# bergmanlab/TELR

Measured on AMD Instinct MI355X. Metric: gbp_aligned_per_s, higher is better.
Workload: dtype int16

## Files before the change

telr_amd/csrc/kernels.hip.h:

```cpp
#pragma once
#include <hip/hip_runtime.h>
#include <stdint.h>

#define TELR_NEG      (-(1 << 28))
#include "part_plan.h"
#define SK_TILE       1024
#define SK_THREADS    256
#define DP_DMAX       4096

struct ChainOpt {
    int32_t max_gap, bw, min_cnt, min_chain_score, chain_gap_q8, chain_skip_q8;
    int32_t dense_n, dense_span, mw_n;
};
struct DpOpt {
    int32_t a, b, q, e, q2, e2, sc_ambi, zdrop;
    int32_t cx_scale, cx_open, cx_emax, cx_emin, cx_dec, cx_flat;
};
__host__ __device__ __forceinline__ int d_cx_ext(const DpOpt &o, int len) { int v = o.cx_emax - o.cx_dec * len; return v > o.cx_emin ? v : o.cx_emin; }
__host__ __device__ __forceinline__ int d_cx_cost(const DpOpt &o, int L)
{
    int t = o.cx_open;
    for (int i = 0; i < L && i < o.cx_flat; ++i) t += d_cx_ext(o, i);
    if (L > o.cx_flat) t += (L - o.cx_flat) * o.cx_emin;
    return t;
// ... 1563 lines not shown
            const uint32_t qi = (klo >> 8) & 0xffffffu, sp = klo & 0xffu;
            const int32_t gpos = (int32_t)(gi & 0x7fffffffu);
            const int lo = i - CHAIN_SCAN_H > 0 ? i - CHAIN_SCAN_H : 0;
            int32_t best = (int32_t)sp, bp = -1, nskip = 0;
            for (int c = 0; ; ++c) {
                const int jt = i - 1 - 64 * c, j = jt - lane;
                if (jt < lo) break;
                uint32_t g = wg, q = wq; int32_t fj2p2 = wf, pj = wp; bool mk = false;
                if (c > 0 && j >= lo) {
                    const uint64_t k = a[j];
                    g = (uint32_t)(k >> 32); q = (uint32_t)A_Q(k);
                    fj2p2 = 2 * f[base + j] + 2;
                    const int32_t pa = p[base + j];
                    pj = pa >= 0 ? pa - pdelta : -1;
                    mk = mark[base + j] == (int32_t)(base + i);
                }
                const bool inw = j >= lo && ((g ^ gi) >> 31) == 0u && gpos - (int32_t)(g & 0x7fffffffu) <= (int32_t)max_gap;
                bool ok;
                const int32_t v2 = d_chain_link<SKIP>(gi, qi, sp - 1u, g + 1u, q + 1u, fj2p2, max_gap, ddc, gap_q8, skip_q8, ok);
                const bool valid = inw && ok;
                const int32_t v = v2 >> 1;
                const uint32_t u = valid && v > best ? (uint32_t)(v - best) : 0u;
                const uint32_t pre = d_wave_scan_max0(u);
                const uint32_t ex = (uint32_t)__shfl_up((int)pre, 1);
                const bool imp = u > (lane ? ex : 0u);
                fl[lane] = 0;
                const int tl = jt - pj;
                if (valid && pj >= 0 && tl < 64) fl[tl] = 1;
                __builtin_amdgcn_fence(__ATOMIC_SEQ_CST, "wavefront");
                mk = mk || fl[lane] != 0;
                __builtin_amdgcn_fence(__ATOMIC_SEQ_CST, "wavefront");
                const int32_t s = valid ? (imp ? -1 : (mk ? 1 : 0)) : 0;
                const int32_t T = nskip + (int32_t)d_wave_scan_add((uint32_t)s);
                const int32_t x = T + (int32_t)d_wave_scan_max0(T < 0 ? (uint32_t)(-T) : 0u);
                const uint64_t brk = __ballot(x > CHAIN_SCAN_SKIP);
                const int b = brk ? __ffsll((unsigned long long)brk) - 1 : 64;
                const uint64_t scanned = b == 64 ? ~0ULL : ((1ULL << b) - 1);
                const uint64_t im = __ballot(imp) & scanned;
                if (im) {
                    const int hl = 63 - __clzll((long long)im);
                    best += (int32_t)__builtin_amdgcn_readlane((int)u, hl);
                    bp = jt - hl;
                }
                const uint64_t win = __ballot(inw);
                const bool more = b == 64 && win == ~0ULL && jt - 64 >= lo;
                if (!more) break;
                if (valid && pj >= 0 && tl >= 64) mark[base + pj] = (int32_t)(base + i);
                nskip = __builtin_amdgcn_readlane(x, 63);
                __threadfence_block();
            }
            of = lane == ii ? best : of; op = lane == ii ? bp : op;
            wg = (uint32_t)__shfl_up((int)wg, 1); wq = (uint32_t)__shfl_up((int)wq, 1); wf = __shfl_up(wf, 1); wp = __shfl_up(wp, 1);
            if (lane == 0) { wg = gi; wq = qi; wf = 2 * best + 2; wp = bp; }
        }
        if (lane < m) {
            f[base + i0 + lane] = of; p[base + i0 + lane] = op >= 0 ? op + pdelta : -1;
            mark[base + i0 + lane] = -1;
        }
        __threadfence_block();
        kb = kn;
    }
}
template <bool SKIP>
__global__ void __launch_bounds__(64) k_chain_scan(const uint64_t *__restrict__ keys, const int32_t *__restrict__ q_aoff, int32_t nq,
                                                   ChainOpt o, int32_t *__restrict__ f, int32_t *__restrict__ p, int32_t *__restrict__ mark,
                                                   const int32_t *__restrict__ q_order)
{
    __shared__ uint8_t fl[64];
    if ((int)blockIdx.x >= nq) return;
    const int q = q_order ? q_order[blockIdx.x] : blockIdx.x;
    d_chain_run_scan<SKIP>(keys, q_aoff[q], q_aoff[q + 1] - q_aoff[q], 0, o, f, p, mark, fl);
}
template <bool SKIP>
__global__ void __launch_bounds__(64) k_chain_scan_isl(const uint64_t *__restrict__ keys, const int32_t *__restrict__ isl_off, const int32_t *__restrict__ isl_pd,
                                                       const int32_t *__restrict__ nisl, ChainOpt o, int32_t *__restrict__ f, int32_t *__restrict__ p,
                                                       int32_t *__restrict__ mark)
{
    __shared__ uint8_t fl[64];
    const int n_isl = *nisl;
    for (int s = blockIdx.x; s < n_isl; s += gridDim.x)
        d_chain_run_scan<SKIP>(keys, isl_off[s], isl_off[s + 1] - isl_off[s], isl_pd[s], o, f, p, mark, fl);
}

__global__ void k_nonpeak(const int32_t *__restrict__ q_aoff, const int32_t *__restrict__ f, const int32_t *__restrict__ p, uint8_t *__restrict__ nonpeak)
{
    const int q = blockIdx.x;
    const int64_t base = q_aoff[q]; const int n = q_aoff[q + 1] - q_aoff[q];
    for (int i = threadIdx.x; i < n; i += blockDim.x) {
        int pj = p[base + i];
        if (pj >= 0 && f[base + i] > f[base + pj]) nonpeak[base + pj] = 1;
    }
}
__global__ void k_peaks(const int32_t *__restrict__ q_aoff, const int32_t *__restrict__ f, const uint8_t *__restrict__ nonpeak,
                        int32_t min_sc, uint64_t *__restrict__ pk, int32_t *__restrict__ n_peaks, int32_t *__restrict__ pk_end)
{
    __shared__ int32_t cnt;
    const int q = blockIdx.x;
    const int64_t base = q_aoff[q]; const int n = q_aoff[q + 1] - q_aoff[q];
    if (threadIdx.x == 0) cnt = 0;
    __syncthreads();
    for (int i = threadIdx.x; i < n; i += blockDim.x) {
        if (!nonpeak[base + i] && f[base + i] >= min_sc) {
            int s = atomicAdd(&cnt, 1);
            pk[base + s] = (uint64_t)(uint32_t)(0x7fffffff - f[base + i]) << 32 | (uint32_t)i;
        }
    }
    __syncthreads();
    if (threadIdx.x == 0) { n_peaks[q] = cnt; pk_end[q] = (int32_t)base + cnt; }
}

struct ChainRec { int32_t score, cnt, a_off, pad; uint64_t a0, a1; };


#define BT_INF 0xffffffffu
#define BT_RING 512
#define BT_RING_SCAN 8192
__global__ void k_bt_rank(const int32_t *__restrict__ q_aoff, const uint64_t *__restrict__ pk, const int32_t *__restrict__ n_peaks, uint32_t *__restrict__ owner)
{
    const int q = blockIdx.x;
    const int64_t base = q_aoff[q]; const int np = n_peaks[q];
    for (int t = threadIdx.x; t < np; t += blockDim.x) owner[base + (uint32_t)(pk[base + t] & 0xffffffffu)] = (uint32_t)t;
}
template <int RING>
__global__ void __launch_bounds__(64) k_bt_owner(const int32_t *__restrict__ q_aoff, int32_t nq, const int32_t *__restrict__ p, int32_t lookback,
                                                 uint32_t *__restrict__ owner, const int32_t *__restrict__ q_order)
{
    __shared__ uint32_t W[RING];
    __shared__ int32_t UP[64];
    const int q = q_order ? q_order[blockIdx.x] : blockIdx.x, lane = threadIdx.x;
    const int64_t base = q_aoff[q]; const int n = q_aoff[q + 1] - q_aoff[q];
    if (n <= 0) return;
    const int nblk = (n + 63) >> 6;
    for (int blk = nblk - 1; blk >= 0; --blk) {
        const int b0 = blk << 6;
        if (blk == nblk - 1) { for (int x = b0 - lookback + lane; x < b0 + 64; x += 64) if (x >= 0 && x < n) W[x & (RING - 1)] = owner[base + x]; }
        else { const int x = b0 - lookback + lane; if (x >= 0) W[x & (RING - 1)] = owner[base + x]; }
        const int i = b0 + lane; const bool valid = i < n;
        const int pi = valid ? p[base + i] : -1;
        int up = pi >= b0 ? pi - b0 : -1;
        UP[lane] = up;
        for (int k = 0; k < 6; ++k) {
            if (__ballot(up >= 0) == 0) break;
            if (up >= 0) atomicMin(&W[(b0 + up) & (RING - 1)], W[i & (RING - 1)]);
            const int nup = up >= 0 ? UP[up] : -1;
            UP[lane] = nup; up = nup;
        }
        if (valid) {
            const uint32_t v = W[i & (RING - 1)];
            owner[base + i] = v;
            if (pi >= 0 && pi < b0) atomicMin(&W[pi & (RING - 1)], v);
        }
    }
}
template <int RING>
__global__ void __launch_bounds__(64) k_bt_depth(const int32_t *__restrict__ q_aoff, int32_t nq, const int32_t *__restrict__ p, const uint32_t *__restrict__ owner,
                                                 int32_t *__restrict__ depth, int32_t *__restrict__ ch_top, const int32_t *__restrict__ q_order)
{
    __shared__ uint32_t OWN[RING];
    __shared__ int32_t DEP[RING];
    __shared__ int32_t UP[64], VAL[64];
    const int q = q_order ? q_order[blockIdx.x] : blockIdx.x, lane = threadIdx.x;
    const int64_t base = q_aoff[q]; const int n = q_aoff[q + 1] - q_aoff[q];
    const int nblk = (n + 63) >> 6;
    for (int blk = 0; blk < nblk; ++blk) {
        const int b0 = blk << 6, i = b0 + lane; const bool valid = i < n;
        const uint32_t o = valid ? owner[base + i] : BT_INF;
        const int pi = valid ? p[base + i] : -1;
        OWN[i & (RING - 1)] = o;
        const uint32_t po = pi >= 0 ? OWN[pi & (RING - 1)] : BT_INF;
        const bool conn = o != BT_INF && pi >= 0 && po == o;
        int up = -1, val = 0;
        if (conn) { if (pi >= b0) { up = pi - b0; val = 1; } else val = DEP[pi & (RING - 1)] + 1; }
        UP[lane] = up; VAL[lane] = val;
        for (int k = 0; k < 6; ++k) {
            if (__ballot(up >= 0) == 0) break;
            const int add = up >= 0 ? VAL[up] : 0, nup = up >= 0 ? UP[up] : -1;
            val += add;
            VAL[lane] = val; UP[lane] = nup; up = nup;
        }
        DEP[i & (RING - 1)] = val;
        if (valid) {
            depth[base + i] = val;
            if (o != BT_INF && !conn) ch_top[base + o] = i;
        }
    }
}
__global__ void __launch_bounds__(64) k_bt_emit(const uint64_t *__restrict__ keys, const int32_t *__restrict__ q_aoff, int32_t nq, const int32_t *__restrict__ f,
                                                const int32_t *__restrict__ p, const uint64_t *__restrict__ pk, const int32_t *__restrict__ n_peaks,
                                                const int32_t *__restrict__ ch_off, int32_t min_sc, int32_t min_cnt, const uint32_t *__restrict__ owner,
                                                const int32_t *__restrict__ depth, const int32_t *__restrict__ ch_top, int32_t *__restrict__ ch_aoff,
                                                ChainRec *__restrict__ rec, int32_t *__restrict__ n_chains, const int32_t *__restrict__ q_order)
{
    const int q = q_order ? q_order[blockIdx.x] : blockIdx.x, lane = threadIdx.x;
    const int64_t base = q_aoff[q]; const int np = n_peaks[q];
    ChainRec *out = rec + ch_off[q];
    int nch = 0, wr = 0;
    for (int t0 = 0; t0 < np; t0 += 64) {
        const int t = t0 + lane;
        bool keep = false; int cnt = 0, sc = 0, idx = 0, top = 0;
        if (t < np) {
            const uint64_t key = pk[base + t];
            idx = (int)(uint32_t)(key & 0xffffffffu);
            const int fi = 0x7fffffff - (int)(uint32_t)(key >> 32);
            if (owner[base + idx] == (uint32_t)t) {
                cnt = depth[base + idx] + 1;
                top = ch_top[base + t];
                const int pj = p[base + top];
                sc = fi - (pj >= 0 ? f[base + pj] : 0);
                keep = sc >= min_sc && cnt >= min_cnt;
            }
        }
        const uint64_t km = __ballot(keep);
        const int before = __popcll(km & ((1ULL << lane) - 1));
        int ps = keep ? cnt : 0;
#pragma unroll
        for (int d = 1; d < 64; d <<= 1) { const int v = __shfl_up(ps, d); if (lane >= d) ps += v; }
        if (t < np) ch_aoff[base + t] = keep ? wr + ps - cnt : -1;
        if (keep) {
            ChainRec r; r.score = sc; r.cnt = cnt; r.a_off = wr + ps - cnt; r.pad = 0;
            r.a0 = keys[base + top]; r.a1 = keys[base + idx];
            out[nch + before] = r;
        }
        nch += __popcll(km); wr += __shfl(ps, 63);
    }
    if (lane == 0) n_chains[q] = nch;
}
__global__ void k_bt_scatter(const uint64_t *__restrict__ keys, const int32_t *__restrict__ q_aoff, const uint32_t *__restrict__ owner, const int32_t *__restrict__ depth,
                             const int32_t *__restrict__ ch_aoff, uint64_t *__restrict__ canch, const int32_t *__restrict__ q_order)
{
    const int q = q_order ? q_order[blockIdx.x] : blockIdx.x;
    const int64_t base = q_aoff[q]; const int n = q_aoff[q + 1] - q_aoff[q];
    for (int i = threadIdx.x; i < n; i += blockDim.x) {
        const uint32_t o = owner[base + i];
        if (o == BT_INF) continue;
        const int ao = ch_aoff[base + o];
        if (ao >= 0) canch[base + ao + depth[base + i]] = keys[base + i];
    }
}

struct KeptChain {
    int32_t qid, tid, rev, cnt;
    int64_t a_glob;
    int32_t rs, qs, re, qe;
    int32_t qlen, tlen;
    int64_t qbase, tbase;
    uint32_t goff; int32_t pad;
};

struct SelOpt { float mask_level, pri_ratio; int32_t best_n, secondary, per_target; };
struct KeptLite { int32_t qid, score, cnt, rev, tid, rs, re, qs, qe, pad; };
__global__ void k_sel_keys(const int32_t *__restrict__ ch_off, const int32_t *__restrict__ n_chains, const ChainRec *__restrict__ rec,
                           uint64_t *__restrict__ key, int32_t *__restrict__ seg_end)
{
    const int q = blockIdx.x;
    const int base = ch_off[q], n = n_chains[q];
    for (int c = threadIdx.x; c < n; c += blockDim.x) key[base + c] = (uint64_t)(uint32_t)(0x7fffffff - rec[base + c].score) << 32 | (uint32_t)c;
    if (threadIdx.x == 0) seg_end[q] = base + n;
}
__device__ __forceinline__ void d_chain_box(const ChainRec &r, const uint32_t *__restrict__ goff, int n_targets, int &rev, int &tid, int &rs, int &re, int &qs, int &qe)
{
    rev = (int)(r.a0 >> 63);
    tid = d_tid_of(goff, n_targets, (uint32_t)A_G(r.a0));
    const int go = (int)goff[tid];
    rs = A_G(r.a0) - go - A_SPAN(r.a0) + 1; re = A_G(r.a1) - go + 1;
    if (rs < 0) rs = 0;
    qs = A_Q(r.a0) - A_SPAN(r.a0) + 1;      qe = A_Q(r.a1) + 1;
}
#define SEL_PCAP 1024
__global__ void __launch_bounds__(64) k_select1(const int32_t *__restrict__ ch_off, const int32_t *__restrict__ n_chains, const ChainRec *__restrict__ rec,
                                                const uint64_t *__restrict__ skey, const int32_t *__restrict__ qlen_of, const uint32_t *__restrict__ goff, int32_t n_targets,
                                                SelOpt o, int32_t *__restrict__ pfs, int32_t *__restrict__ pfe, int32_t *__restrict__ ptid, int32_t *__restrict__ pkey,
                                                int32_t *__restrict__ tcnt_t, int32_t *__restrict__ tcnt_n, uint8_t *__restrict__ keep, int32_t *__restrict__ n_kept,
                                                const int32_t *__restrict__ q_order)
{
    __shared__ int32_t Lfs[SEL_PCAP], Lfe[SEL_PCAP], Ltid[SEL_PCAP], Lkey[SEL_PCAP];
    const int q = q_order ? q_order[blockIdx.x] : blockIdx.x, lane = threadIdx.x;
    const int base = ch_off[q], n = n_chains[q], qlen = qlen_of[q];
    int n_prim = 0, n2_all = 0, n_t = 0, nk = 0;
    for (int i0 = 0; i0 < n; i0 += 64) {
        const int cnt = n - i0 < 64 ? n - i0 : 64;
        int my_fs = 0, my_fe = 0, my_tid = 0, my_sc = 0;
        if (lane < cnt) {
            const ChainRec r = rec[base + (int)(uint32_t)(skey[base + i0 + lane] & 0xffffffffu)];
            int rev, rs, re, qs, qe;
            d_chain_box(r, goff, n_targets, rev, my_tid, rs, re, qs, qe);
            my_fs = rev ? qlen - qe : qs; my_fe = rev ? qlen - qs : qe; my_sc = r.score;
        }
        bool my_keep = false;
        for (int u = 0; u < cnt; ++u) {
            const int fs = __builtin_amdgcn_readlane(my_fs, u), fe = __builtin_amdgcn_readlane(my_fe, u), tid = __builtin_amdgcn_readlane(my_tid, u),
                      sc = __builtin_amdgcn_readlane(my_sc, u);
            int parent = -1;
            for (int c0 = 0; c0 < n_prim && parent < 0; c0 += 64) {
                const int j = c0 + lane;
                bool hit = false;
                if (j < n_prim) {
                    const int jt = j < SEL_PCAP ? Ltid[j] : ptid[base + j];
                    if (!o.per_target || jt == tid) {
                        const int js = j < SEL_PCAP ? Lfs[j] : pfs[base + j], je = j < SEL_PCAP ? Lfe[j] : pfe[base + j];
                        const int lo = fs > js ? fs : js, hi = fe < je ? fe : je;
                        const int ol = hi > lo ? hi - lo : 0;
                        const int mn = (fe - fs) < (je - js) ? (fe - fs) : (je - js);
                        hit = (float)ol > o.mask_level * (float)mn;
                    }
                }
                const uint64_t m = __ballot(hit);
                if (m) parent = c0 + __ffsll((unsigned long long)m) - 1;
            }
            bool kp;
            if (parent < 0) {
                if (lane == 0) {
                    if (n_prim < SEL_PCAP) { Lfs[n_prim] = fs; Lfe[n_prim] = fe; Ltid[n_prim] = tid; Lkey[n_prim] = sc; }
                    else { pfs[base + n_prim] = fs; pfe[base + n_prim] = fe; ptid[base + n_prim] = tid; pkey[base + n_prim] = sc; }
                }
// ... 1916 lines not shown
```

telr_amd/csrc/telr_engine.hip:

```cpp
#include <hip/hip_runtime.h>
#include <cstring>
#include <string.h>
#include <rocprim/rocprim.hpp>
#include <algorithm>
#include <atomic>
#include <immintrin.h>
#include <chrono>
#include <cmath>
#include <condition_variable>
#include <cstdio>
#include <cstdlib>
#include <cstring>
#include <map>
#include <memory>
#include <mutex>
#include <string>
#include <thread>
#include <sys/mman.h>
#include <vector>
#include "../../include/telr_hip.h"
#include "kernels.hip.h"
#include "range_plan.h"
#include "sam_records.h"
#define TELR_HAVE_SEED_ARGS 1
// ... 1486 lines not shown
                          int32_t n_over, const int32_t *d_overlist, const int32_t *d_qorder, int32_t *d_f, int32_t *d_p)
{
    ChainOpt co; co.max_gap = mo->max_gap; co.bw = mo->bw_long > mo->bw ? mo->bw_long : mo->bw; co.min_cnt = mo->min_cnt; co.min_chain_score = mo->min_chain_score;
    co.chain_gap_q8 = mo->chain_gap_q8; co.chain_skip_q8 = mo->chain_skip_q8;
    static const bool chain_push = ab_on("chain_push"), chain_lazy = ab_on("chain_lazy"), chain_no_mw = ab_on("chain_no_mw");
    static int dense_v[3] = {2048, 48, 1 << 19};
    static const bool dense_env = [] { if (const char *e = getenv("TELR_CHAIN_DENSE")) sscanf(e, "%d%*[,:]%d%*[,:]%d", &dense_v[0], &dense_v[1], &dense_v[2]); return true; }();
    (void)dense_env;
    const int Rr = mo->chain_lookback / 64;
    const bool mw_all = dense_v[2] <= SEGSORT_CAP;
    static const bool no_islands = ab_on("no_islands");
    const bool islands = nq <= CHAIN_ISL_NQ && na > 0 && !no_islands;
    const bool mw = !(mo->flags & TELR_MF_CHAIN_SKIP) && !chain_push && !chain_lazy && !chain_no_mw && Rr >= 2 && na > 0 && !islands && dense_v[2] > 0 && (mw_all || n_over > 0);
    co.dense_n = dense_v[0]; co.dense_span = dense_v[1]; co.mw_n = mw ? dense_v[2] : 0;
#define CHAIN_LAUNCH(RR, SK) do { if (chain_push) hipLaunchKernelGGL((k_chain<RR, SK, 0>), dim3(nq), dim3(64), 0, st, d_skeys, d_qaoff, nq, co, d_f, d_p, d_qorder, 0); \
                                  else if (chain_lazy) hipLaunchKernelGGL((k_chain<RR, SK, 1>), dim3(nq), dim3(64), 0, st, d_skeys, d_qaoff, nq, co, d_f, d_p, d_qorder, 0); \
                                  else hipLaunchKernelGGL((k_chain<RR, SK, 2>), dim3(nq), dim3(64), 0, st, d_skeys, d_qaoff, nq, co, d_f, d_p, d_qorder, mw ? 1 : 0); } while (0)
#define CHAIN_MW(RR, SK) hipLaunchKernelGGL((k_chain_mw<RR, SK>), dim3(mw_all ? nq : n_over), dim3(64 * RR), 0, ctx->side[0], d_skeys, d_qaoff, mw_all ? nq : n_over, mw_all ? (const int32_t*)nullptr : (const int32_t*)d_overlist, co, d_f, d_p)
    const bool skip = co.chain_skip_q8 != 0;
    if (mo->flags & TELR_MF_CHAIN_SKIP) {
        int32_t *d_mark;
        TRY(ctx_buf_t(ctx, "chain_mark", (size_t)na + 1, &d_mark));
        if (islands) {
            int32_t *d_head, *d_rank, *d_ioff, *d_ipd;
            TRY(ctx_buf_t(ctx, "isl_head", (size_t)na + 1, &d_head));
            TRY(ctx_buf_t(ctx, "isl_rank", (size_t)na + 1, &d_rank));
            TRY(ctx_buf_t(ctx, "isl_off", (size_t)na + 2, &d_ioff));
            TRY(ctx_buf_t(ctx, "isl_pd", (size_t)na + 1, &d_ipd));
            HIPCHK(hipMemsetAsync(d_head + na, 0, 4, st));
            hipLaunchKernelGGL(k_isl_heads, dim3(nq), dim3(256), 0, st, d_skeys, d_qaoff, nq, (uint32_t)co.max_gap, d_head);
            HIPCHK(hipGetLastError());
            TRY((dev_exclusive_scan<int32_t, int32_t>(ctx, d_head, d_rank, (size_t)na + 1)));
            hipLaunchKernelGGL(k_isl_fill, dim3(nq), dim3(256), 0, st, d_qaoff, nq, d_head, d_rank, (int32_t)na, d_ioff, d_ipd);
            const unsigned grid = (unsigned)std::min<int64_t>((int64_t)na, 256 * 32);
            if (skip) hipLaunchKernelGGL(k_chain_scan_isl<true>, dim3(grid), dim3(64), 0, st, d_skeys, d_ioff, d_ipd, d_rank + na, co, d_f, d_p, d_mark);
            else hipLaunchKernelGGL(k_chain_scan_isl<false>, dim3(grid), dim3(64), 0, st, d_skeys, d_ioff, d_ipd, d_rank + na, co, d_f, d_p, d_mark);
        } else if (nq > 0) {
            if (skip) hipLaunchKernelGGL(k_chain_scan<true>, dim3(nq), dim3(64), 0, st, d_skeys, d_qaoff, nq, co, d_f, d_p, d_mark, d_qorder);
            else hipLaunchKernelGGL(k_chain_scan<false>, dim3(nq), dim3(64), 0, st, d_skeys, d_qaoff, nq, co, d_f, d_p, d_mark, d_qorder);
        }
        HIPCHK(hipGetLastError());
        return TELR_OK;
    }
    if (islands) {
        int32_t *d_head, *d_rank, *d_ioff, *d_ipd;
        TRY(ctx_buf_t(ctx, "isl_head", (size_t)na + 1, &d_head));
        TRY(ctx_buf_t(ctx, "isl_rank", (size_t)na + 1, &d_rank));
        TRY(ctx_buf_t(ctx, "isl_off", (size_t)na + 2, &d_ioff));
        TRY(ctx_buf_t(ctx, "isl_pd", (size_t)na + 1, &d_ipd));
        HIPCHK(hipMemsetAsync(d_head + na, 0, 4, st));
        hipLaunchKernelGGL(k_isl_heads, dim3(nq), dim3(256), 0, st, d_skeys, d_qaoff, nq, (uint32_t)co.max_gap, d_head);
        HIPCHK(hipGetLastError());
        TRY((dev_exclusive_scan<int32_t, int32_t>(ctx, d_head, d_rank, (size_t)na + 1)));
        hipLaunchKernelGGL(k_isl_fill, dim3(nq), dim3(256), 0, st, d_qaoff, nq, d_head, d_rank, (int32_t)na, d_ioff, d_ipd);
        const unsigned grid = (unsigned)std::min<int64_t>((int64_t)na, 256 * 32);
#define CHAIN_ISL(RR, SK) do { if (chain_push) hipLaunchKernelGGL((k_chain_isl<RR, SK, 0>), dim3(grid), dim3(64), 0, st, d_skeys, d_ioff, d_ipd, d_rank + na, co, d_f, d_p); \
                               else if (chain_lazy) hipLaunchKernelGGL((k_chain_isl<RR, SK, 1>), dim3(grid), dim3(64), 0, st, d_skeys, d_ioff, d_ipd, d_rank + na, co, d_f, d_p); \
                               else hipLaunchKernelGGL((k_chain_isl<RR, SK, 2>), dim3(grid), dim3(64), 0, st, d_skeys, d_ioff, d_ipd, d_rank + na, co, d_f, d_p); } while (0)
        if (Rr == 1) { if (skip) CHAIN_ISL(1, true); else CHAIN_ISL(1, false); }
        else if (Rr == 2) { if (skip) CHAIN_ISL(2, true); else CHAIN_ISL(2, false); }
        else { if (skip) CHAIN_ISL(4, true); else CHAIN_ISL(4, false); }
#undef CHAIN_ISL
    }
    else {
        if (mw) {
            HIPCHK(hipEventRecord(ctx->ev_side[0], st));
            HIPCHK(hipStreamWaitEvent(ctx->side[0], ctx->ev_side[0], 0));
            if (Rr == 2) { if (skip) CHAIN_MW(2, true); else CHAIN_MW(2, false); }
            else { if (skip) CHAIN_MW(4, true); else CHAIN_MW(4, false); }
            HIPCHK(hipEventRecord(ctx->ev_side[0], ctx->side[0]));
        }
        if (Rr == 1) { if (skip) CHAIN_LAUNCH(1, true); else CHAIN_LAUNCH(1, false); }
        else if (Rr == 2) { if (skip) CHAIN_LAUNCH(2, true); else CHAIN_LAUNCH(2, false); }
        else { if (skip) CHAIN_LAUNCH(4, true); else CHAIN_LAUNCH(4, false); }
        if (mw) HIPCHK(hipStreamWaitEvent(st, ctx->ev_side[0], 0));
    }
#undef CHAIN_LAUNCH
#undef CHAIN_MW
    HIPCHK(hipGetLastError());
    return TELR_OK;
}

struct BtOut { uint64_t *d_canch; int32_t *d_choff, *d_nch; ChainRec *d_rec; int32_t npk_tot; };
static int backtrack_dispatch(telr_ctx *ctx, hipStream_t st, const telr_map_opt *mo, const uint64_t *d_skeys, const int32_t *d_qaoff, int nq, int32_t na,
                              bool any_over, const int32_t *d_qorder, const int32_t *d_f, const int32_t *d_p, BtOut *out)
{
    uint8_t *d_flags; uint64_t *d_pk, *d_pk2, *d_canch; int32_t *d_npk, *d_pkend, *d_choff, *d_nch;
    TRY(ctx_buf_t(ctx, "flags", (size_t)na + 16, &d_flags));
    uint8_t *d_nonpeak = d_flags;
    TRY(ctx_buf_t(ctx, "pk", (size_t)na, &d_pk));
    TRY(ctx_buf_t(ctx, "pk2", (size_t)na, &d_pk2));
    TRY(ctx_buf_t(ctx, "canch", (size_t)na, &d_canch));
    TRY(ctx_buf_t(ctx, "n_peaks", (size_t)nq + 1, &d_npk));
    TRY(ctx_buf_t(ctx, "pk_end", (size_t)nq + 1, &d_pkend));
    TRY(ctx_buf_t(ctx, "ch_off", (size_t)nq + 1, &d_choff));
    TRY(ctx_buf_t(ctx, "n_chains", (size_t)nq + 1, &d_nch));
    HIPCHK(hipMemsetAsync(d_flags, 0, (size_t)na + 16, st));
    hipLaunchKernelGGL(k_nonpeak, dim3(nq), dim3(256), 0, st, d_qaoff, d_f, d_p, d_nonpeak);
    hipLaunchKernelGGL(k_peaks, dim3(nq), dim3(256), 0, st, d_qaoff, d_f, d_nonpeak, mo->min_chain_score, d_pk, d_npk, d_pkend);
    HIPCHK(hipGetLastError());
    if (na > 0) TRY(seg_sort_u64(ctx, "so_p", d_pk, d_pk2, d_qaoff, d_pkend, nullptr, d_qorder, nq, (size_t)na, any_over, st));
    HIPCHK(hipMemsetAsync(d_npk + nq, 0, 4, st));
    TRY((dev_exclusive_scan<int32_t, int32_t>(ctx, d_npk, d_choff, (size_t)nq + 1)));
    int32_t npk_tot = 0;
    HIPCHK(hipMemcpyAsync(&npk_tot, d_choff + nq, 4, hipMemcpyDeviceToHost, st));
    HIPCHK(hipStreamSynchronize(st));
    ChainRec *d_rec;
    TRY(ctx_buf_t(ctx, "chain_rec", (size_t)npk_tot, &d_rec));
    {
        uint32_t *d_owner; int32_t *d_depth, *d_chtop, *d_chaoff;
        TRY(ctx_buf_t(ctx, "bt_owner", (size_t)na + 1, &d_owner));
        TRY(ctx_buf_t(ctx, "bt_depth", (size_t)na + 1, &d_depth));
        TRY(ctx_buf_t(ctx, "bt_chtop", (size_t)na + 1, &d_chtop));
        TRY(ctx_buf_t(ctx, "bt_chaoff", (size_t)na + 1, &d_chaoff));
        HIPCHK(hipMemsetAsync(d_owner, 0xff, ((size_t)na + 1) * 4, st));
        hipLaunchKernelGGL(k_bt_rank, dim3(nq), dim3(256), 0, st, d_qaoff, d_pk2, d_npk, d_owner);
        if (mo->flags & TELR_MF_CHAIN_SKIP) {
            hipLaunchKernelGGL(k_bt_owner<BT_RING_SCAN>, dim3(nq), dim3(64), 0, st, d_qaoff, nq, d_p, (int32_t)CHAIN_SCAN_H, d_owner, d_qorder);
            hipLaunchKernelGGL(k_bt_depth<BT_RING_SCAN>, dim3(nq), dim3(64), 0, st, d_qaoff, nq, d_p, d_owner, d_depth, d_chtop, d_qorder);
        } else {
            hipLaunchKernelGGL(k_bt_owner<BT_RING>, dim3(nq), dim3(64), 0, st, d_qaoff, nq, d_p, mo->chain_lookback, d_owner, d_qorder);
            hipLaunchKernelGGL(k_bt_depth<BT_RING>, dim3(nq), dim3(64), 0, st, d_qaoff, nq, d_p, d_owner, d_depth, d_chtop, d_qorder);
        }
        hipLaunchKernelGGL(k_bt_emit, dim3(nq), dim3(64), 0, st, d_skeys, d_qaoff, nq, d_f, d_p, d_pk2, d_npk, d_choff, mo->min_chain_score, mo->min_cnt,
                           d_owner, d_depth, d_chtop, d_chaoff, d_rec, d_nch, d_qorder);
        hipLaunchKernelGGL(k_bt_scatter, dim3(nq), dim3(256), 0, st, d_skeys, d_qaoff, d_owner, d_depth, d_chaoff, d_canch, d_qorder);
        HIPCHK(hipGetLastError());
    }
    HIPCHK(hipGetLastError());
    out->d_canch = d_canch; out->d_choff = d_choff; out->d_nch = d_nch; out->d_rec = d_rec; out->npk_tot = npk_tot;
    return TELR_OK;
}

struct SelOut { int nk; KeptLite *hl; KeptChain *d_kc; const uint64_t *d_sk2; const uint8_t *d_keep; };
static int select1_dispatch(telr_ctx *ctx, hipStream_t st, const telr_map_opt *mo, const int32_t *d_choff, const int32_t *d_nch, const ChainRec *d_rec, int32_t npk_tot,
                            const int32_t *d_qaoff, int nq, int32_t q0, const int32_t *d_qlen, const int64_t *d_qboff, const uint32_t *d_goff, const int32_t *d_tlen,
                            const int64_t *d_tboff, int32_t n_targets, bool any_over, const int32_t *d_qorder, bool need_recs, int32_t *h_nch, int32_t *q_k0, SelOut *out)
{
    uint64_t *d_sk, *d_sk2; int32_t *d_segend, *d_pfs, *d_pfe, *d_ptid, *d_pkey, *d_tct, *d_tcn, *d_nkept, *d_koff; uint8_t *d_keep;
    TRY(ctx_buf_t(ctx, "sel_key", (size_t)npk_tot + 1, &d_sk));
    TRY(ctx_buf_t(ctx, "sel_key2", (size_t)npk_tot + 1, &d_sk2));
    TRY(ctx_buf_t(ctx, "sel_segend", (size_t)nq + 1, &d_segend));
    TRY(ctx_buf_t(ctx, "sel_pfs", (size_t)npk_tot + 1, &d_pfs));
    TRY(ctx_buf_t(ctx, "sel_pfe", (size_t)npk_tot + 1, &d_pfe));
    TRY(ctx_buf_t(ctx, "sel_ptid", (size_t)npk_tot + 1, &d_ptid));
    TRY(ctx_buf_t(ctx, "sel_pkey", (size_t)npk_tot + 1, &d_pkey));
    TRY(ctx_buf_t(ctx, "sel_tct", (size_t)npk_tot + 1, &d_tct));
    TRY(ctx_buf_t(ctx, "sel_tcn", (size_t)npk_tot + 1, &d_tcn));
    TRY(ctx_buf_t(ctx, "sel_keep", (size_t)npk_tot + 1, &d_keep));
    TRY(ctx_buf_t(ctx, "sel_nkept", (size_t)nq + 2, &d_nkept));
    TRY(ctx_buf_t(ctx, "sel_koff", (size_t)nq + 2, &d_koff));
    hipLaunchKernelGGL(k_sel_keys, dim3(nq), dim3(64), 0, st, d_choff, d_nch, d_rec, d_sk, d_segend);
    HIPCHK(hipGetLastError());
    if (npk_tot > 0) TRY(seg_sort_u64(ctx, "so_c", d_sk, d_sk2, d_choff, d_segend, nullptr, d_qorder, nq, (size_t)npk_tot, any_over, st));
    SelOpt so; so.mask_level = mo->mask_level; so.pri_ratio = mo->pri_ratio; so.best_n = mo->best_n; so.secondary = mo->secondary;
    so.per_target = (mo->flags & TELR_MF_PER_TARGET) ? 1 : 0;
    hipLaunchKernelGGL(k_select1, dim3(nq), dim3(64), 0, st, d_choff, d_nch, d_rec, d_sk2, d_qlen, d_goff, n_targets, so,
                       d_pfs, d_pfe, d_ptid, d_pkey, d_tct, d_tcn, d_keep, d_nkept, d_qorder);
    HIPCHK(hipGetLastError());
    HIPCHK(hipMemsetAsync(d_nkept + nq, 0, 4, st));
    TRY((dev_exclusive_scan<int32_t, int32_t>(ctx, d_nkept, d_koff, (size_t)nq + 1)));
    HIPCHK(hipMemcpyAsync(q_k0, d_koff, (size_t)(nq + 1) * 4, hipMemcpyDeviceToHost, st));
    if (!need_recs) HIPCHK(hipMemcpyAsync(h_nch, d_nch, (size_t)nq * 4, hipMemcpyDeviceToHost, st));
    HIPCHK(hipStreamSynchronize(st));
    const int nk = q_k0[nq];
    KeptLite *d_kl;
    KeptChain *d_kc; KeptLite *hl;
    TRY(ctx_buf_t(ctx, "kept", (size_t)nk, &d_kc));
    TRY(ctx_buf_t(ctx, "kept_lite", (size_t)nk, &d_kl));
    TRY(ctx_hbuf_t(ctx, "h_kept_lite", (size_t)nk, &hl));
    if (nk > 0) {
        hipLaunchKernelGGL(k_select1_write, dim3(nq), dim3(64), 0, st, d_choff, d_nch, d_rec, d_sk2, d_keep, d_koff, d_qaoff, q0, d_qlen, d_qboff,
                           d_goff, d_tlen, d_tboff, n_targets, d_kc, d_kl);
        HIPCHK(hipGetLastError());
        HIPCHK(hipMemcpyAsync(hl, d_kl, (size_t)nk * sizeof(KeptLite), hipMemcpyDeviceToHost, st));
        HIPCHK(hipStreamSynchronize(st));
    }
    out->nk = nk; out->hl = hl; out->d_kc = d_kc; out->d_sk2 = d_sk2; out->d_keep = d_keep;
    return TELR_OK;
}

static int segments_dispatch(telr_ctx *ctx, hipStream_t st, const telr_map_opt *mo, const KeptChain *d_kc, int nk, const uint64_t *d_canch,
                             std::vector<int32_t> &h_poff, int *np_out, DpProb **d_probs_out)
{
    int32_t *d_nprob, *d_poff;
    TRY(ctx_buf_t(ctx, "nprob", (size_t)nk + 1, &d_nprob));
    TRY(ctx_buf_t(ctx, "prob_off", (size_t)nk + 1, &d_poff));
    hipLaunchKernelGGL(k_segments_w<0>, dim3(nk), dim3(64), 0, st, d_kc, nk, d_canch, mo->min_ksw_len, mo->bw, mo->fill_band_q4, mo->ext_max, mo->ext_band, mo->bw_long, d_nprob, (const int32_t*)nullptr, (DpProb*)nullptr);
    HIPCHK(hipGetLastError());
    HIPCHK(hipMemsetAsync(d_nprob + nk, 0, 4, st));
    TRY((dev_exclusive_scan<int32_t, int32_t>(ctx, d_nprob, d_poff, (size_t)nk + 1)));
    h_poff.resize(nk + 1);
    HIPCHK(hipMemcpyAsync(h_poff.data(), d_poff, (size_t)(nk + 1) * 4, hipMemcpyDeviceToHost, st));
    HIPCHK(hipStreamSynchronize(st));
    const int np = h_poff[nk];
    DpProb *d_probs;
    TRY(ctx_buf_t(ctx, "probs", (size_t)np, &d_probs));
    hipLaunchKernelGGL(k_segments_w<1>, dim3(nk), dim3(64), 0, st, d_kc, nk, d_canch, mo->min_ksw_len, mo->bw, mo->fill_band_q4, mo->ext_max, mo->ext_band, mo->bw_long, d_nprob, d_poff, d_probs);
    HIPCHK(hipGetLastError());
    *np_out = np; *d_probs_out = d_probs;
    return TELR_OK;
}

static void chain_row(const ChainRec &r, int32_t qid, const uint32_t *goff, int n_targets, int32_t *v)
{
    const uint32_t g0 = (uint32_t)A_G(r.a0);
    const int tid = (int)(std::upper_bound(goff, goff + n_targets, g0) - goff) - 1, go = (int)goff[tid];
    v[0] = qid; v[1] = r.score; v[2] = r.cnt; v[3] = (int)(r.a0 >> 63); v[4] = tid;
    v[5] = std::max(0, A_G(r.a0) - go - A_SPAN(r.a0) + 1);
    v[6] = A_G(r.a1) - go + 1; v[7] = A_Q(r.a0) - A_SPAN(r.a0) + 1; v[8] = A_Q(r.a1) + 1;
}


struct QueryOrder {
    int32_t *d = nullptr, *h = nullptr; std::thread t;
    ~QueryOrder() { if (t.joinable()) t.join(); }
};
static int query_order_start(telr_ctx *ctx, const telr_seqset *qs, int32_t q0, int nq, QueryOrder *o)
{
    TRY(ctx_hbuf_t(ctx, "h_qorder", (size_t)nq + 1, &o->h));
    TRY(ctx_buf_t(ctx, "q_order", (size_t)nq + 1, &o->d));
    int32_t *h_ord = o->h;
    o->t = std::thread([=]() {
        for (int i = 0; i < nq; ++i) h_ord[i] = i;
        std::stable_sort(h_ord, h_ord + nq, [&](int32_t x, int32_t y) { return qs->len[q0 + x] > qs->len[q0 + y]; });
    });
    return TELR_OK;
}
static int query_order_upload(telr_ctx *ctx, hipStream_t st, int nq, QueryOrder *o)
{
    o->t.join();
    HIPCHK(hipMemcpyAsync(o->d, o->h, (size_t)nq * 4, hipMemcpyHostToDevice, st));
    return TELR_OK;
}

// ... 1096 lines not shown
```

Baseline: 21.84.

## Fuse chain back-tracking peak finding, sort, owner and depth sweeps into one kernel

Adds k_bt_find, which finds peaks per query in a single wavefront, sorts them with an in-LDS bitonic sort, then runs the owner and depth sweeps without leaving the block. k_bt_write merges chain emission, scatter and selection-key generation. Queries that are too long or have too many peaks are routed to the original multi-kernel path through a fall-back list. The aim is to remove several launches, a global segmented sort, memsets and global round-trips. The cost is heavier per-block work, a large LDS footprint and a second host sync when fall-backs occur.

```diff
diff --git a/telr_amd/csrc/kernels.hip.h b/telr_amd/csrc/kernels.hip.h
--- a/telr_amd/csrc/kernels.hip.h
+++ b/telr_amd/csrc/kernels.hip.h
@@ -1669,9 +1669,10 @@
         d_chain_run_scan<SKIP>(keys, isl_off[s], isl_off[s + 1] - isl_off[s], isl_pd[s], o, f, p, mark, fl);
 }
 
-__global__ void k_nonpeak(const int32_t *__restrict__ q_aoff, const int32_t *__restrict__ f, const int32_t *__restrict__ p, uint8_t *__restrict__ nonpeak)
-{
-    const int q = blockIdx.x;
+__global__ void k_nonpeak(const int32_t *__restrict__ q_aoff, const int32_t *__restrict__ f, const int32_t *__restrict__ p, uint8_t *__restrict__ nonpeak,
+                          const int32_t *__restrict__ list)
+{
+    const int q = list ? list[blockIdx.x] : blockIdx.x;
     const int64_t base = q_aoff[q]; const int n = q_aoff[q + 1] - q_aoff[q];
     for (int i = threadIdx.x; i < n; i += blockDim.x) {
         int pj = p[base + i];
@@ -1679,10 +1680,10 @@
     }
 }
 __global__ void k_peaks(const int32_t *__restrict__ q_aoff, const int32_t *__restrict__ f, const uint8_t *__restrict__ nonpeak,
-                        int32_t min_sc, uint64_t *__restrict__ pk, int32_t *__restrict__ n_peaks, int32_t *__restrict__ pk_end)
+                        int32_t min_sc, uint64_t *__restrict__ pk, int32_t *__restrict__ n_peaks, int32_t *__restrict__ pk_end, const int32_t *__restrict__ list)
 {
     __shared__ int32_t cnt;
-    const int q = blockIdx.x;
+    const int q = list ? list[blockIdx.x] : blockIdx.x;
     const int64_t base = q_aoff[q]; const int n = q_aoff[q + 1] - q_aoff[q];
     if (threadIdx.x == 0) cnt = 0;
     __syncthreads();
@@ -1702,9 +1703,10 @@
 #define BT_INF 0xffffffffu
 #define BT_RING 512
 #define BT_RING_SCAN 8192
-__global__ void k_bt_rank(const int32_t *__restrict__ q_aoff, const uint64_t *__restrict__ pk, const int32_t *__restrict__ n_peaks, uint32_t *__restrict__ owner)
-{
-    const int q = blockIdx.x;
+__global__ void k_bt_rank(const int32_t *__restrict__ q_aoff, const uint64_t *__restrict__ pk, const int32_t *__restrict__ n_peaks, uint32_t *__restrict__ owner,
+                          const int32_t *__restrict__ list)
+{
+    const int q = list ? list[blockIdx.x] : blockIdx.x;
     const int64_t base = q_aoff[q]; const int np = n_peaks[q];
     for (int t = threadIdx.x; t < np; t += blockDim.x) owner[base + (uint32_t)(pk[base + t] & 0xffffffffu)] = (uint32_t)t;
 }
@@ -1817,6 +1819,194 @@
 {
     const int q = q_order ? q_order[blockIdx.x] : blockIdx.x;
     const int64_t base = q_aoff[q]; const int n = q_aoff[q + 1] - q_aoff[q];
+    for (int i = threadIdx.x; i < n; i += blockDim.x) {
+        const uint32_t o = owner[base + i];
+        if (o == BT_INF) continue;
+        const int ao = ch_aoff[base + o];
+        if (ao >= 0) canch[base + ao + depth[base + i]] = keys[base + i];
+    }
+}
+
+#define BT_PKCAP 1008
+__device__ __forceinline__ void d_bt_cswap(uint64_t *PK, int a, int b, int n)
+{
+    if (b < n) { const uint64_t x = PK[a], y = PK[b]; if (x > y) { PK[a] = y; PK[b] = x; } }
+}
+template <int RING>
+__global__ void __launch_bounds__(64) k_bt_find(const int32_t *__restrict__ q_aoff, int32_t nq, const int32_t *__restrict__ f, const int32_t *__restrict__ p,
+                                                int32_t lookback, int32_t min_sc, int32_t n_cap, uint64_t *__restrict__ pk2, int32_t *__restrict__ n_peaks,
+                                                int32_t *__restrict__ pk_end, int32_t *__restrict__ fb_end, uint32_t *owner, int32_t *__restrict__ depth,
+                                                int32_t *__restrict__ ch_top, const int32_t *__restrict__ q_order, int32_t *__restrict__ fb_cnt,
+                                                int32_t *__restrict__ fb_list)
+{
+    constexpr int P1 = 2 * BT_PKCAP + RING + RING / 32, P3 = 2 * RING + 128, NW = P1 > P3 ? P1 : P3;
+    __shared__ uint64_t L64[(NW + 1) / 2];
+    uint32_t *const L = (uint32_t*)L64;
+    if ((int)blockIdx.x >= nq) return;
+    const int q = q_order ? q_order[blockIdx.x] : blockIdx.x, lane = threadIdx.x;
+    const int64_t base = q_aoff[q]; const int n = q_aoff[q + 1] - q_aoff[q];
+    if (lane == 0) fb_end[q] = (int32_t)base;
+    if (n > n_cap) { if (lane == 0) { fb_list[atomicAdd(fb_cnt, 1)] = q; n_peaks[q] = 0; } return; }
+    uint64_t *const PK = L64;
+    int32_t *const F = (int32_t*)(L + 2 * BT_PKCAP);
+    uint32_t *const NPW = L + 2 * BT_PKCAP + RING;
+    const int nblk = (n + 63) >> 6, lag = (lookback + 63) >> 6;
+    int cnt = 0;
+    auto retire = [&](int k) {
+        const int j = (k << 6) + lane, r = j & (RING - 1);
+        const int fj = F[r];
+        const bool is_pk = j < n && !(NPW[r >> 5] >> (r & 31) & 1u) && fj >= min_sc;
+        const uint64_t m = __ballot(is_pk);
+        const int s = cnt + __popcll(m & ((1ULL << lane) - 1));
+        if (is_pk && s < BT_PKCAP) PK[s] = (uint64_t)(uint32_t)(0x7fffffff - fj) << 32 | (uint32_t)j;
+        if (j < n && !is_pk) owner[base + j] = BT_INF;
+        cnt += __popcll(m);
+    };
+    int fi_n = lane < n ? f[base + lane] : 0, pi_n = lane < n ? p[base + lane] : -1;
+    for (int b = 0; b < nblk; ++b) {
+        const int i = (b << 6) + lane, r = i & (RING - 1);
+        const int fi = fi_n, pi = pi_n;
+        { const int i2 = i + 64; const bool v2 = i2 < n; fi_n = v2 ? f[base + i2] : 0; pi_n = v2 ? p[base + i2] : -1; }
+        F[r] = fi;
+        if (lane < 2) NPW[(r >> 5) + lane] = 0;
+        __builtin_amdgcn_wave_barrier();
+        if (pi >= 0 && fi > F[pi & (RING - 1)]) atomicOr(&NPW[(pi & (RING - 1)) >> 5], 1u << (pi & 31));
+        __builtin_amdgcn_wave_barrier();
+        if (b >= lag) retire(b - lag);
+    }
+    for (int k = nblk > lag ? nblk - lag : 0; k < nblk; ++k) retire(k);
+    if (cnt > BT_PKCAP) { if (lane == 0) { fb_list[atomicAdd(fb_cnt, 1)] = q; n_peaks[q] = 0; } return; }
+    __syncthreads();
+    int half = 1;
+    while (2 * half < cnt) half <<= 1;
+    for (int k = 2; (k >> 1) < cnt; k <<= 1) {
+        for (int x = lane; x < half; x += 64) { const int a = (x / (k >> 1)) * k + (x & ((k >> 1) - 1)); d_bt_cswap(PK, a, a ^ (k - 1), cnt); }
+        __syncthreads();
+        for (int j = k >> 2; j > 0; j >>= 1) {
+            for (int x = lane; x < half; x += 64) { const int a = ((x & ~(j - 1)) << 1) | (x & (j - 1)); d_bt_cswap(PK, a, a | j, cnt); }
+            __syncthreads();
+        }
+    }
+    for (int t = lane; t < cnt; t += 64) {
+        const uint64_t key = PK[t];
+        pk2[base + t] = key;
+        owner[base + (uint32_t)(key & 0xffffffffu)] = (uint32_t)t;
+    }
+    if (lane == 0) { n_peaks[q] = cnt; pk_end[q] = (int32_t)base + cnt; }
+    __syncthreads();
+    if (n <= 0) return;
+    {
+        uint32_t *const W = L; int32_t *const UP = (int32_t*)(L + RING);
+        int pi_n = ((nblk - 1) << 6) + lane < n ? p[base + ((nblk - 1) << 6) + lane] : -1;
+        uint32_t w_n = BT_INF;
+        for (int blk = nblk - 1; blk >= 0; --blk) {
+            const int b0 = blk << 6;
+            if (blk == nblk - 1) { for (int x = b0 - lookback + lane; x < b0 + 64; x += 64) if (x >= 0 && x < n) W[x & (RING - 1)] = owner[base + x]; }
+            else { const int x = b0 - lookback + lane; if (x >= 0) W[x & (RING - 1)] = w_n; }
+            const int i = b0 + lane; const bool valid = i < n;
+            const int pi = pi_n;
+            if (blk > 0) {
+                const int x2 = b0 - 64 - lookback + lane;
+                w_n = x2 >= 0 ? owner[base + x2] : BT_INF;
+                pi_n = p[base + i - 64];
+            }
+            int up = pi >= b0 ? pi - b0 : -1;
+            UP[lane] = up;
+            for (int k = 0; k < 6; ++k) {
+                if (__ballot(up >= 0) == 0) break;
+                if (up >= 0) atomicMin(&W[(b0 + up) & (RING - 1)], W[i & (RING - 1)]);
+                const int nup = up >= 0 ? UP[up] : -1;
+                UP[lane] = nup; up = nup;
+            }
+            if (valid) {
+                const uint32_t v = W[i & (RING - 1)];
+                owner[base + i] = v;
+                if (pi >= 0 && pi < b0) atomicMin(&W[pi & (RING - 1)], v);
+            }
+        }
+    }
+    __syncthreads();
+    {
+        uint32_t *const OWN = L; int32_t *const DEP = (int32_t*)(L + RING), *const UP = (int32_t*)(L + 2 * RING), *const VAL = (int32_t*)(L + 2 * RING + 64);
+        uint32_t o_n = lane < n ? owner[base + lane] : BT_INF;
+        int pi_n = lane < n ? p[base + lane] : -1;
+        for (int blk = 0; blk < nblk; ++blk) {
+            const int b0 = blk << 6, i = b0 + lane; const bool valid = i < n;
+            const uint32_t o = o_n;
+            const int pi = pi_n;
+            { const int i2 = i + 64; const bool v2 = i2 < n; o_n = v2 ? owner[base + i2] : BT_INF; pi_n = v2 ? p[base + i2] : -1; }
+            OWN[i & (RING - 1)] = o;
+            const uint32_t po = pi >= 0 ? OWN[pi & (RING - 1)] : BT_INF;
+            const bool conn = o != BT_INF && pi >= 0 && po == o;
+            int up = -1, val = 0;
+            if (conn) { if (pi >= b0) { up = pi - b0; val = 1; } else val = DEP[pi & (RING - 1)] + 1; }
+            UP[lane] = up; VAL[lane] = val;
+            for (int k = 0; k < 6; ++k) {
+                if (__ballot(up >= 0) == 0) break;
+                const int add = up >= 0 ? VAL[up] : 0, nup = up >= 0 ? UP[up] : -1;
+                val += add;
+                VAL[lane] = val; UP[lane] = nup; up = nup;
+            }
+            DEP[i & (RING - 1)] = val;
+            if (valid) {
+                depth[base + i] = val;
+                if (o != BT_INF && !conn) ch_top[base + o] = i;
+            }
+        }
+    }
+}
+__global__ void k_bt_fb_init(const int32_t *__restrict__ q_aoff, const int32_t *__restrict__ list, uint8_t *__restrict__ nonpeak, uint32_t *__restrict__ owner)
+{
+    const int q = list[blockIdx.x];
+    const int64_t base = q_aoff[q]; const int n = q_aoff[q + 1] - q_aoff[q];
+    for (int i = threadIdx.x; i < n; i += blockDim.x) { nonpeak[base + i] = 0; owner[base + i] = BT_INF; }
+}
+__global__ void __launch_bounds__(256) k_bt_write(const uint64_t *__restrict__ keys, const int32_t *__restrict__ q_aoff, int32_t nq, const int32_t *__restrict__ f,
+                                                  const int32_t *__restrict__ p, const uint64_t *__restrict__ pk, const int32_t *__restrict__ n_peaks,
+                                                  const int32_t *__restrict__ ch_off, int32_t min_sc, int32_t min_cnt, const uint32_t *__restrict__ owner,
+                                                  const int32_t *__restrict__ depth, const int32_t *__restrict__ ch_top, int32_t *ch_aoff,
+                                                  ChainRec *__restrict__ rec, int32_t *__restrict__ n_chains, uint64_t *__restrict__ skey,
+                                                  int32_t *__restrict__ seg_end, uint64_t *__restrict__ canch, const int32_t *__restrict__ q_order)
+{
+    if ((int)blockIdx.x >= nq) return;
+    const int q = q_order ? q_order[blockIdx.x] : blockIdx.x;
+    const int64_t base = q_aoff[q]; const int n = q_aoff[q + 1] - q_aoff[q];
+    if (threadIdx.x < 64) {
+        const int lane = threadIdx.x, np = n_peaks[q], c0 = ch_off[q];
+        ChainRec *out = rec + c0;
+        int nch = 0, wr = 0;
+        for (int t0 = 0; t0 < np; t0 += 64) {
+            const int t = t0 + lane;
+            bool keep = false; int cnt = 0, sc = 0, idx = 0, top = 0;
+            if (t < np) {
+                const uint64_t key = pk[base + t];
+                idx = (int)(uint32_t)(key & 0xffffffffu);
+                const int fi = 0x7fffffff - (int)(uint32_t)(key >> 32);
+                if (owner[base + idx] == (uint32_t)t) {
+                    cnt = depth[base + idx] + 1;
+                    top = ch_top[base + t];
+                    const int pj = p[base + top];
+                    sc = fi - (pj >= 0 ? f[base + pj] : 0);
+                    keep = sc >= min_sc && cnt >= min_cnt;
+                }
+            }
+            const uint64_t km = __ballot(keep);
+            const int before = __popcll(km & ((1ULL << lane) - 1));
+            int ps = keep ? cnt : 0;
+#pragma unroll
+            for (int d = 1; d < 64; d <<= 1) { const int v = __shfl_up(ps, d); if (lane >= d) ps += v; }
+            if (t < np) ch_aoff[base + t] = keep ? wr + ps - cnt : -1;
+            if (keep) {
+                ChainRec r; r.score = sc; r.cnt = cnt; r.a_off = wr + ps - cnt; r.pad = 0;
+                r.a0 = keys[base + top]; r.a1 = keys[base + idx];
+                out[nch + before] = r;
+                skey[c0 + nch + before] = (uint64_t)(uint32_t)(0x7fffffff - sc) << 32 | (uint32_t)(nch + before);
+            }
+            nch += __popcll(km); wr += __shfl(ps, 63);
+        }
+        if (lane == 0) { n_chains[q] = nch; seg_end[q] = c0 + nch; }
+    }
+    __syncthreads();
     for (int i = threadIdx.x; i < n; i += blockDim.x) {
         const uint32_t o = owner[base + i];
         if (o == BT_INF) continue;
diff --git a/telr_amd/csrc/telr_engine.hip b/telr_amd/csrc/telr_engine.hip
--- a/telr_amd/csrc/telr_engine.hip
+++ b/telr_amd/csrc/telr_engine.hip
@@ -1592,6 +1592,13 @@
 }
 
 struct BtOut { uint64_t *d_canch; int32_t *d_choff, *d_nch; ChainRec *d_rec; int32_t npk_tot; };
+static bool bt_fused(const telr_map_opt *mo)
+{
+    static const bool unfused = ab_on("bt_unfused");
+    const bool skip = (mo->flags & TELR_MF_CHAIN_SKIP) != 0;
+    const int look = skip ? (int)CHAIN_SCAN_H : mo->chain_lookback;
+    return !unfused && look >= 0 && ((look + 63) / 64 + 1) * 64 <= (skip ? BT_RING_SCAN : BT_RING);
+}
 static int backtrack_dispatch(telr_ctx *ctx, hipStream_t st, const telr_map_opt *mo, const uint64_t *d_skeys, const int32_t *d_qaoff, int nq, int32_t na,
                               bool any_over, const int32_t *d_qorder, const int32_t *d_f, const int32_t *d_p, BtOut *out)
 {
@@ -1601,41 +1608,83 @@
     TRY(ctx_buf_t(ctx, "pk", (size_t)na, &d_pk));
     TRY(ctx_buf_t(ctx, "pk2", (size_t)na, &d_pk2));
     TRY(ctx_buf_t(ctx, "canch", (size_t)na, &d_canch));
-    TRY(ctx_buf_t(ctx, "n_peaks", (size_t)nq + 1, &d_npk));
+    TRY(ctx_buf_t(ctx, "n_peaks", (size_t)nq + 2, &d_npk));
     TRY(ctx_buf_t(ctx, "pk_end", (size_t)nq + 1, &d_pkend));
     TRY(ctx_buf_t(ctx, "ch_off", (size_t)nq + 1, &d_choff));
     TRY(ctx_buf_t(ctx, "n_chains", (size_t)nq + 1, &d_nch));
-    HIPCHK(hipMemsetAsync(d_flags, 0, (size_t)na + 16, st));
-    hipLaunchKernelGGL(k_nonpeak, dim3(nq), dim3(256), 0, st, d_qaoff, d_f, d_p, d_nonpeak);
-    hipLaunchKernelGGL(k_peaks, dim3(nq), dim3(256), 0, st, d_qaoff, d_f, d_nonpeak, mo->min_chain_score, d_pk, d_npk, d_pkend);
-    HIPCHK(hipGetLastError());
-    if (na > 0) TRY(seg_sort_u64(ctx, "so_p", d_pk, d_pk2, d_qaoff, d_pkend, nullptr, d_qorder, nq, (size_t)na, any_over, st));
-    HIPCHK(hipMemsetAsync(d_npk + nq, 0, 4, st));
-    TRY((dev_exclusive_scan<int32_t, int32_t>(ctx, d_npk, d_choff, (size_t)nq + 1)));
-    int32_t npk_tot = 0;
-    HIPCHK(hipMemcpyAsync(&npk_tot, d_choff + nq, 4, hipMemcpyDeviceToHost, st));
-    HIPCHK(hipStreamSynchronize(st));
+    uint32_t *d_owner; int32_t *d_depth, *d_chtop, *d_chaoff;
+    TRY(ctx_buf_t(ctx, "bt_owner", (size_t)na + 1, &d_owner));
+    TRY(ctx_buf_t(ctx, "bt_depth", (size_t)na + 1, &d_depth));
+    TRY(ctx_buf_t(ctx, "bt_chtop", (size_t)na + 1, &d_chtop));
+    TRY(ctx_buf_t(ctx, "bt_chaoff", (size_t)na + 1, &d_chaoff));
+    const bool fused = bt_fused(mo), skip = (mo->flags & TELR_MF_CHAIN_SKIP) != 0;
+    const int32_t look = skip ? (int32_t)CHAIN_SCAN_H : mo->chain_lookback;
+    auto sweeps = [&](const int32_t *list, int n) {
+        hipLaunchKernelGGL(k_bt_rank, dim3(n), dim3(256), 0, st, d_qaoff, d_pk2, d_npk, d_owner, list);
+        const int32_t *ord = list ? list : d_qorder;
+        if (skip) {
+            hipLaunchKernelGGL(k_bt_owner<BT_RING_SCAN>, dim3(n), dim3(64), 0, st, d_qaoff, nq, d_p, look, d_owner, ord);
+            hipLaunchKernelGGL(k_bt_depth<BT_RING_SCAN>, dim3(n), dim3(64), 0, st, d_qaoff, nq, d_p, d_owner, d_depth, d_chtop, ord);
+        } else {
+            hipLaunchKernelGGL(k_bt_owner<BT_RING>, dim3(n), dim3(64), 0, st, d_qaoff, nq, d_p, look, d_owner, ord);
+            hipLaunchKernelGGL(k_bt_depth<BT_RING>, dim3(n), dim3(64), 0, st, d_qaoff, nq, d_p, d_owner, d_depth, d_chtop, ord);
+        }
+    };
+    int32_t npk_tot = 0, n_fb = 0;
+    auto scan_peaks = [&]() -> int {
+        TRY((dev_exclusive_scan<int32_t, int32_t>(ctx, d_npk, d_choff, (size_t)nq + 1)));
+        HIPCHK(hipMemcpyAsync(&npk_tot, d_choff + nq, 4, hipMemcpyDeviceToHost, st));
+        if (fused) HIPCHK(hipMemcpyAsync(&n_fb, d_npk + nq + 1, 4, hipMemcpyDeviceToHost, st));
+        HIPCHK(hipStreamSynchronize(st));
+        return TELR_OK;
+    };
+    if (fused) {
+        int32_t *d_fbend, *d_fblist;
+        TRY(ctx_buf_t(ctx, "bt_fbend", (size_t)nq + 1, &d_fbend));
+        TRY(ctx_buf_t(ctx, "bt_fblist", (size_t)nq + 1, &d_fblist));
+        HIPCHK(hipMemsetAsync(d_npk + nq, 0, 8, st));
+        if (skip) hipLaunchKernelGGL(k_bt_find<BT_RING_SCAN>, dim3(nq), dim3(64), 0, st, d_qaoff, nq, d_f, d_p, look, mo->min_chain_score, (int32_t)SEGSORT_CAP, d_pk2, d_npk, d_pkend, d_fbend,
+                                     d_owner, d_depth, d_chtop, d_qorder, d_npk + nq + 1, d_fblist);
+        else hipLaunchKernelGGL(k_bt_find<BT_RING>, dim3(nq), dim3(64), 0, st, d_qaoff, nq, d_f, d_p, look, mo->min_chain_score, (int32_t)SEGSORT_CAP, d_pk2, d_npk, d_pkend, d_fbend,
+                                d_owner, d_depth, d_chtop, d_qorder, d_npk + nq + 1, d_fblist);
+        HIPCHK(hipGetLastError());
+        TRY(scan_peaks());
+        if (n_fb < 0 || n_fb > nq) { ctx->err = "back-tracking: fall-back count outside the range"; return TELR_E_RANGE; }
+        if (n_fb > 0) {
+            hipLaunchKernelGGL(k_bt_fb_init, dim3(n_fb), dim3(256), 0, st, d_qaoff, d_fblist, d_nonpeak, d_owner);
+            hipLaunchKernelGGL(k_nonpeak, dim3(n_fb), dim3(256), 0, st, d_qaoff, d_f, d_p, d_nonpeak, d_fblist);
+            hipLaunchKernelGGL(k_peaks, dim3(n_fb), dim3(256), 0, st, d_qaoff, d_f, d_nonpeak, mo->min_chain_score, d_pk, d_npk, d_fbend, d_fblist);
+            HIPCHK(hipGetLastError());
+            TRY(seg_sort_u64(ctx, "so_p", d_pk, d_pk2, d_qaoff, d_fbend, nullptr, d_qorder, nq, (size_t)na, any_over, st));
+            sweeps(d_fblist, n_fb);
+            HIPCHK(hipGetLastError());
+            TRY(scan_peaks());
+        }
+        static const bool trace = trace_on("bt");
+        if (trace) fprintf(stderr, "[telr bt] %d queries, %d anchors: %d took the fall-back launches\n", nq, na, n_fb);
+    } else {
+        HIPCHK(hipMemsetAsync(d_flags, 0, (size_t)na + 16, st));
+        hipLaunchKernelGGL(k_nonpeak, dim3(nq), dim3(256), 0, st, d_qaoff, d_f, d_p, d_nonpeak, (const int32_t*)nullptr);
+        hipLaunchKernelGGL(k_peaks, dim3(nq), dim3(256), 0, st, d_qaoff, d_f, d_nonpeak, mo->min_chain_score, d_pk, d_npk, d_pkend, (const int32_t*)nullptr);
+        HIPCHK(hipGetLastError());
+        if (na > 0) TRY(seg_sort_u64(ctx, "so_p", d_pk, d_pk2, d_qaoff, d_pkend, nullptr, d_qorder, nq, (size_t)na, any_over, st));
+        HIPCHK(hipMemsetAsync(d_npk + nq, 0, 4, st));
+        TRY(scan_peaks());
+    }
     ChainRec *d_rec;
     TRY(ctx_buf_t(ctx, "chain_rec", (size_t)npk_tot, &d_rec));
-    {
-        uint32_t *d_owner; int32_t *d_depth, *d_chtop, *d_chaoff;
-        TRY(ctx_buf_t(ctx, "bt_owner", (size_t)na + 1, &d_owner));
-        TRY(ctx_buf_t(ctx, "bt_depth", (size_t)na + 1, &d_depth));
-        TRY(ctx_buf_t(ctx, "bt_chtop", (size_t)na + 1, &d_chtop));
-        TRY(ctx_buf_t(ctx, "bt_chaoff", (size_t)na + 1, &d_chaoff));
+    if (fused) {
+        uint64_t *d_sk; int32_t *d_segend;
+        TRY(ctx_buf_t(ctx, "sel_key", (size_t)npk_tot + 1, &d_sk));
+        TRY(ctx_buf_t(ctx, "sel_segend", (size_t)nq + 1, &d_segend));
+        hipLaunchKernelGGL(k_bt_write, dim3(nq), dim3(256), 0, st, d_skeys, d_qaoff, nq, d_f, d_p, d_pk2, d_npk, d_choff, mo->min_chain_score, mo->min_cnt,
+                           d_owner, d_depth, d_chtop, d_chaoff, d_rec, d_nch, d_sk, d_segend, d_canch, d_qorder);
+    } else {
         HIPCHK(hipMemsetAsync(d_owner, 0xff, ((size_t)na + 1) * 4, st));
-        hipLaunchKernelGGL(k_bt_rank, dim3(nq), dim3(256), 0, st, d_qaoff, d_pk2, d_npk, d_owner);
-        if (mo->flags & TELR_MF_CHAIN_SKIP) {
-            hipLaunchKernelGGL(k_bt_owner<BT_RING_SCAN>, dim3(nq), dim3(64), 0, st, d_qaoff, nq, d_p, (int32_t)CHAIN_SCAN_H, d_owner, d_qorder);
-            hipLaunchKernelGGL(k_bt_depth<BT_RING_SCAN>, dim3(nq), dim3(64), 0, st, d_qaoff, nq, d_p, d_owner, d_depth, d_chtop, d_qorder);
-        } else {
-            hipLaunchKernelGGL(k_bt_owner<BT_RING>, dim3(nq), dim3(64), 0, st, d_qaoff, nq, d_p, mo->chain_lookback, d_owner, d_qorder);
-            hipLaunchKernelGGL(k_bt_depth<BT_RING>, dim3(nq), dim3(64), 0, st, d_qaoff, nq, d_p, d_owner, d_depth, d_chtop, d_qorder);
-        }
+        sweeps(nullptr, nq);
         hipLaunchKernelGGL(k_bt_emit, dim3(nq), dim3(64), 0, st, d_skeys, d_qaoff, nq, d_f, d_p, d_pk2, d_npk, d_choff, mo->min_chain_score, mo->min_cnt,
                            d_owner, d_depth, d_chtop, d_chaoff, d_rec, d_nch, d_qorder);
         hipLaunchKernelGGL(k_bt_scatter, dim3(nq), dim3(256), 0, st, d_skeys, d_qaoff, d_owner, d_depth, d_chaoff, d_canch, d_qorder);
-        HIPCHK(hipGetLastError());
     }
     HIPCHK(hipGetLastError());
     out->d_canch = d_canch; out->d_choff = d_choff; out->d_nch = d_nch; out->d_rec = d_rec; out->npk_tot = npk_tot;
@@ -1660,7 +1709,7 @@
     TRY(ctx_buf_t(ctx, "sel_keep", (size_t)npk_tot + 1, &d_keep));
     TRY(ctx_buf_t(ctx, "sel_nkept", (size_t)nq + 2, &d_nkept));
     TRY(ctx_buf_t(ctx, "sel_koff", (size_t)nq + 2, &d_koff));
-    hipLaunchKernelGGL(k_sel_keys, dim3(nq), dim3(64), 0, st, d_choff, d_nch, d_rec, d_sk, d_segend);
+    if (!bt_fused(mo)) hipLaunchKernelGGL(k_sel_keys, dim3(nq), dim3(64), 0, st, d_choff, d_nch, d_rec, d_sk, d_segend);
     HIPCHK(hipGetLastError());
     if (npk_tot > 0) TRY(seg_sort_u64(ctx, "so_c", d_sk, d_sk2, d_choff, d_segend, nullptr, d_qorder, nq, (size_t)npk_tot, any_over, st));
     SelOpt so; so.mask_level = mo->mask_level; so.pri_ratio = mo->pri_ratio; so.best_n = mo->best_n; so.secondary = mo->secondary;
```

Result: no change. 21.77 (-0.3%).
